# meco-group/omg-tools

Measured on AMD Instinct MI355X. Metric: MPC solves/sec, 1024-agent Holonomic Point2point batch per GPU, higher is better.
Workload: dtype f64

## Files before the change

### omg-tools_amd/csrc/omgx_core.h

```cpp
#pragma once
#include <stdint.h>
#include <math.h>

#ifdef OMGX_HOST_PORT
#define OMGX_FN inline
#define OMGX_HD inline
#else
#define OMGX_FN __device__ __forceinline__
#define OMGX_HD __host__ __device__ inline
#endif

#ifdef OMGX_HOST_PORT
#include <vector>
static thread_local std::vector<double> omgx_rbak;
#endif
#ifdef OMGX_COUNT_FACT
#include <atomic>
static std::atomic<long> omgx_dbg_nfact(0);
static std::atomic<long> omgx_dbg_cnt[12];
#endif
namespace omgx {

enum { ROW_FREE = 0, ROW_UPPER = 1, ROW_LOWER = 2, ROW_EQ = 3, ROW_BAD = 4 };
enum { OP_DIV = 0, OP_BSPL = 1, OP_COS = 2, OP_SIN = 3 };
// ... 207 lines not shown
  *lds = nl; *hbm = ng;
}

OMGX_HD size_t work_doubles(const Dims& d, int kkt_doubles) {
  size_t nl, ng;
  work_split(d, kkt_doubles, WS_LDS, &nl, &ng);
  return nl;
}

template <int MODE>
OMGX_HD void work_carve_split(Work& w, double* lds, double* hbm, const Dims& d, int kkt_doubles) {
  double* p = lds;
  double* g = hbm;
  w.slots = p; p += d.n_slots;
  if (!d.atoms_alias) { w.atoms = p; p += d.n_atoms; w.knots = p; p += d.n_knots; }
  w.x = p; p += d.N;             w.xt = p; p += d.N;
  w.gbar = p; p += d.N;          w.sol = p; p += d.N + d.n_eq;
  if (d.atoms_alias) { w.atoms = w.gbar; w.knots = w.gbar + d.n_atoms; }
  w.dinv = p; p += d.N;
  w.red = p; p += 64;
  if (ws_rows_hbm(MODE)) {
    w.ht = g; g += d.n_con;        w.rho = g; g += d.n_con;     w.vv = g; g += d.n_con;
    w.z = g; g += d.n_con;         w.ds = g; g += d.n_con;
    w.rtype = (int8_t*)g; g += (d.n_con + 7) / 8;
  } else {
    w.ht = p; p += d.n_con;        w.rho = p; p += d.n_con;     w.vv = p; p += d.n_con;
    w.z = p; p += d.n_con;         w.ds = p; p += d.n_con;
    w.rtype = (int8_t*)p; p += (d.n_con + 7) / 8;
  }
  if (ws_hv_hbm(MODE)) { w.hv = g; g += d.n_con; } else { w.hv = p; p += d.n_con; }
  if (ws_jac_hbm(MODE)) { w.jval = g; g += d.nnz_j + 1; } else { w.jval = p; p += d.nnz_j + 1; }
  if (ws_kkt_hbm(MODE)) { w.kkt = g; g += kkt_doubles; w.col = p; p += ws_root_lds(MODE) ? d.col_small : d.col_small_noroot; }
  else { w.kkt = p; p += kkt_doubles; w.col = p; p += d.col_doubles; }
  w.root = ws_root_lds(MODE) ? w.col + (OMGX_BMAT_DOUBLES + OMGX_STAGE_LD) * (OMGX_MAX_LEAF + 1) + OMGX_PAN_LD * (d.nr + 1) : nullptr;
}

OMGX_HD void work_carve(Work& w, double* base, const Dims& d, int kkt_doubles) {
  work_carve_split<WS_LDS>(w, base, nullptr, d, kkt_doubles);
}

#ifdef OMGX_HOST_PORT
struct Ctx {
  static constexpr bool wave_only = false, hbm = false, no_wave = false, root_lds = false, general = true, prep = false, refine = true, lean = false;
  double* red;
  int tid() const { return 0; }
  int nthr() const { return 1; }
  void sync() const {}
  double uni(double v) const { return v; }
  double rsum(double v) const { return v; }
  double wave_sum(double v) const { return v; }
  double rmax(double v) const { return v; }
  double rmin(double v) const { return v; }
  template <int... OPS> void reduce_ops(double (&)[sizeof...(OPS)]) const {}
  int lane() const { return 0; }
  int nlanes() const { return 1; }
  int wave() const { return 0; }
  int nwaves() const { return 1; }
  void wave_sync() const {}
};
#else
template <bool kHbm, bool kWaveOnly = false, bool kRootLds = false, bool kGeneral = false, bool kPrep = false, bool kRefine = false,
          bool kLean = false>
struct CtxT {
  static constexpr bool hbm = kHbm;
  static constexpr bool prep = kPrep;
  static constexpr bool refine = kRefine;
  static constexpr bool lean = kLean;
  static constexpr bool general = kGeneral;
  static constexpr bool root_lds = kRootLds;
  static constexpr bool wave_only = kWaveOnly;
  static constexpr bool no_wave = kHbm;
  double* red;
  long long* prof;
  __device__ int tid() const { int t = threadIdx.x; asm volatile("" : "+v"(t)); return t; }
  __device__ int nthr() const { return blockDim.x; }
  __device__ void sync() const { __syncthreads(); }
  template <int OP> static __device__ __forceinline__ double comb(double a, double b) {
    return OP == 0 ? a + b : (OP == 1 ? fmax(a, b) : fmin(a, b));
  }
  template <int OP, int CTRL> static __device__ __forceinline__ double dpp_comb(double v) {
    const int lo = __double2loint(v), hi = __double2hiint(v);
    const int lo2 = __builtin_amdgcn_update_dpp(lo, lo, CTRL, 0xf, 0xf, false);
    const int hi2 = __builtin_amdgcn_update_dpp(hi, hi, CTRL, 0xf, 0xf, false);
    return comb<OP>(v, __hiloint2double(hi2, lo2));
  }
  template <int OP> static __device__ __forceinline__ double wave_reduce(double v) {
    v = dpp_comb<OP, 0x128>(v);
    v = dpp_comb<OP, 0x124>(v);
    v = dpp_comb<OP, 0x122>(v);
    v = dpp_comb<OP, 0x121>(v);
    const double r0 = rl(v, 0), r1 = rl(v, 16), r2 = rl(v, 32), r3 = rl(v, 48);
    return comb<OP>(comb<OP>(r0, r1), comb<OP>(r2, r3));
  }
  static __device__ __forceinline__ double rl(double v, int lane) {
    return __hiloint2double(__builtin_amdgcn_readlane(__double2hiint(v), lane), __builtin_amdgcn_readlane(__double2loint(v), lane));
  }
  static __device__ __forceinline__ double uni(double v) {
    return __hiloint2double(__builtin_amdgcn_readfirstlane(__double2hiint(v)), __builtin_amdgcn_readfirstlane(__double2loint(v)));
  }
  template <int OP> __device__ double reduce(double v) const {
    v = wave_reduce<OP>(v);
    const int wave = threadIdx.x >> 6, nw = (blockDim.x + 63) >> 6;
    if ((threadIdx.x & 63) == 0) red[wave] = v;
    __syncthreads();
    double r = red[0];
    for (int i = 1; i < nw; ++i) r = comb<OP>(r, red[i]);
    __syncthreads();
    return uni(r);
  }
  template <int I, int N, int OP0, int... OPS>
  __device__ __forceinline__ void red_wave(double (&v)[N]) const {
    v[I] = wave_reduce<OP0>(v[I]);
    if ((threadIdx.x & 63) == 0) red[(threadIdx.x >> 6) * N + I] = v[I];
    if constexpr (sizeof...(OPS) > 0) red_wave<I + 1, N, OPS...>(v);
  }
  template <int I, int N, int OP0, int... OPS>
  __device__ __forceinline__ void red_block(double (&v)[N]) const {
    const int nw = (blockDim.x + 63) >> 6;
    double r = red[I];
    for (int k = 1; k < nw; ++k) r = comb<OP0>(r, red[k * N + I]);
    v[I] = uni(r);
    if constexpr (sizeof...(OPS) > 0) red_block<I + 1, N, OPS...>(v);
  }
  template <int... OPS> __device__ __forceinline__ void reduce_ops(double (&v)[sizeof...(OPS)]) const {
    static_assert(sizeof...(OPS) <= 8, "reduction scratch holds 8 values per wave");
    red_wave<0, sizeof...(OPS), OPS...>(v);
    __syncthreads();
    red_block<0, sizeof...(OPS), OPS...>(v);
    __syncthreads();
  }
  __device__ double rsum(double v) const { return reduce<0>(v); }
  __device__ double wave_sum(double v) const { return wave_reduce<0>(v); }
  __device__ double rmax(double v) const { return reduce<1>(v); }
  __device__ double rmin(double v) const { return reduce<2>(v); }
  __device__ int lane() const { return threadIdx.x & 63; }
  __device__ int nlanes() const { return 64; }
  __device__ int wave() const { return __builtin_amdgcn_readfirstlane(threadIdx.x >> 6); }
  __device__ int nwaves() const { return blockDim.x >> 6; }
  __device__ void wave_sync() const {
    if (kHbm) { __builtin_amdgcn_fence(__ATOMIC_RELEASE, "workgroup"); __builtin_amdgcn_wave_barrier(); __builtin_amdgcn_fence(__ATOMIC_ACQUIRE, "workgroup"); }
    else { __builtin_amdgcn_fence(__ATOMIC_RELEASE, "wavefront"); __builtin_amdgcn_wave_barrier(); __builtin_amdgcn_fence(__ATOMIC_ACQUIRE, "wavefront"); }
  }
};
typedef CtxT<false> Ctx;
#endif

#define OMGX_PFOR(i, n) for (int i = c.tid(); i < (n); i += c.nthr())
#define OMGX_PFOR_U4(i, n) _Pragma("unroll 4") for (int i = c.tid(); i < (n); i += c.nthr())

enum { PH_JAC = 0, PH_RESID, PH_ASSEMBLE, PH_FACTOR, PH_SOLVE, PH_STEP, PH_LINESEARCH, PH_UPDATE, PH_F_LEAF, PH_F_SCHUR, PH_F_ROOT, PH_LA, PH_LS, PH_LB, PH_SETUP, PH_TOTAL,
       PH_S_DESC, PH_S_PARAMS, PH_S_JAC0, PH_S_CLASS, PH_S_INIT, PH_A_ZERO, PH_A_PAIRS, PH_A_REST, PH_A_DIAG,
       PH_K_FWD, PH_K_ROOTRHS, PH_K_ROOT, PH_K_LEAFRHS, PH_K_BWD, PH_L_TERMS, PH_L_ROWS,
       PH_F_PARK, PH_F_SWEEP, PH_F_SCALE, PH_A_TCOL, PH_A_HESS, PH_P_LOAD, PH_P_DIV, PH_P_BSPL, PH_P_SLOTS, PH_COUNT };
#if defined(OMGX_PROFILE) && !defined(OMGX_HOST_PORT)
#define OMGX_TIC() long long tic_ = (c.sync(), clock64())
#define OMGX_TOC(k) do { c.sync(); long long now_ = clock64(); if (c.tid() == 0 && c.prof) c.prof[k] += now_ - tic_; tic_ = now_; } while (0)
#else
#define OMGX_TIC() do {} while (0)
#define OMGX_TOC(k) do {} while (0)
#endif

OMGX_FN double pp_eval(const Tables& T, int pp, const double* a) {
  double tot = 0.0;
  for (int m = T.pp_ptr[pp]; m < T.pp_ptr[pp + 1]; ++m) {
    double v = T.pm_coef[m];
    for (int q = T.pm_ptr[m]; q < T.pm_ptr[m + 1]; ++q) v *= a[T.pm_atom[q]];
    tot += v;
  }
  return tot;
}

OMGX_FN double csr_range_eval(const Tables& T, int m0, int m1, const double* a) {
  double tot = 0.0;
  for (int m = m0; m < m1; ++m) {
    double v = T.pm_coef[m];
    for (int q = T.pm_ptr[m]; q < T.pm_ptr[m + 1]; ++q) v *= a[T.pm_atom[q]];
    tot += v;
  }
  return tot;
}

OMGX_FN double mono_range_eval(const Tables& T, int m0, int m1, const double* a) {
  double tot = 0.0;
#pragma unroll 4
  for (int m = m0; m < m1; ++m) {
    const MonoRec r = T.pm_rec[m];
    double v = r.coef;
    if (r.a0 >= 0) { v *= a[r.a0]; if (r.a1 >= 0) { v *= a[r.a1]; if (r.a2 >= 0) { v *= a[r.a2]; if (r.a3 >= 0) v *= a[r.a3]; } } }
    tot += v;
  }
  return tot;
}

OMGX_FN double pp_eval_packed(const Tables& T, int pp, const double* a) {
  double tot = 0.0;
  const int m0 = T.pp_ptr[pp], m1 = T.pp_ptr[pp + 1];
#pragma unroll 4
  for (int m = m0; m < m1; ++m) {
    const MonoRec r = T.pm_rec[m];
    double v = r.coef;
    if (r.a0 >= 0) { v *= a[r.a0]; if (r.a1 >= 0) { v *= a[r.a1]; if (r.a2 >= 0) { v *= a[r.a2]; if (r.a3 >= 0) v *= a[r.a3]; } } }
    tot += v;
  }
  return tot;
}

template <bool GEN>
OMGX_FN void bspl_row(const double* k, int n_knots, int deg, double u, double* out) {
  const int n_fun = n_knots - deg - 1;
  int j = deg;
  for (int q = deg + 1; q < n_fun; ++q) if (k[q] < u) j = q;
  const bool inside = (u >= k[0]) && (u <= k[n_knots - 1]);
  if (GEN && deg > 5) {
    for (int i = 0; i < n_fun; ++i) out[i] = 0.0;
    if (!inside) return;
    double* Nv = out + (j - deg);
    Nv[0] = 1.0;
    for (int r = 1; r <= deg; ++r) {
      double saved = 0.0;
      for (int q = 0; q < r; ++q) {
        const double rgt = k[j + q + 1] - u, lft = u - k[j + 1 - (r - q)];
        const double den = rgt + lft;
        const double temp = den != 0.0 ? Nv[q] / den : 0.0;
        Nv[q] = saved + rgt * temp;
        saved = lft * temp;
      }
      Nv[r] = saved;
    }
    return;
  }
  double N[6], left[6], right[6];
#pragma unroll
  for (int r = 0; r < 6; ++r) { N[r] = 0.0; left[r] = 0.0; right[r] = 0.0; }
  N[0] = 1.0;
#pragma unroll
  for (int r = 1; r <= 5; ++r) {
    if (r <= deg) {
      left[r] = u - k[j + 1 - r];
      right[r] = k[j + r] - u;
      double saved = 0.0;
#pragma unroll
      for (int q = 0; q < 5; ++q) {
        if (q < r) {
          const double den = right[q + 1] + left[r - q];
          const double temp = den != 0.0 ? N[q] / den : 0.0;
          N[q] = saved + right[q + 1] * temp;
          saved = left[r - q] * temp;
        }
      }
      N[r] = saved;
    }
  }
  for (int i = 0; i < n_fun; ++i) out[i] = 0.0;
#pragma unroll
  for (int r = 0; r < 6; ++r) if (r <= deg && inside) out[j - deg + r] = N[r];
}

OMGX_FN double mono_value(const MonoRec& r, const double* at) {
  const double a0 = at[r.a0 < 0 ? 0 : r.a0], a1 = at[r.a1 < 0 ? 0 : r.a1];
  const double a2 = at[r.a2 < 0 ? 0 : r.a2], a3 = at[r.a3 < 0 ? 0 : r.a3];
  return r.coef * (r.a0 < 0 ? 1.0 : a0) * (r.a1 < 0 ? 1.0 : a1) * (r.a2 < 0 ? 1.0 : a2) * (r.a3 < 0 ? 1.0 : a3);
}
OMGX_FN double mono_value(const MonoRec8& r, const double* at) {
  const double a0 = at[r.a0 < 0 ? 0 : r.a0], a1 = at[r.a1 < 0 ? 0 : r.a1];
  const double a2 = at[r.a2 < 0 ? 0 : r.a2], a3 = at[r.a3 < 0 ? 0 : r.a3];
  const double a4 = at[r.a4 < 0 ? 0 : r.a4], a5 = at[r.a5 < 0 ? 0 : r.a5];
  const double a6 = at[r.a6 < 0 ? 0 : r.a6], a7 = at[r.a7 < 0 ? 0 : r.a7];
  return r.coef * (r.a0 < 0 ? 1.0 : a0) * (r.a1 < 0 ? 1.0 : a1) * (r.a2 < 0 ? 1.0 : a2) * (r.a3 < 0 ? 1.0 : a3)
                * (r.a4 < 0 ? 1.0 : a4) * (r.a5 < 0 ? 1.0 : a5) * (r.a6 < 0 ? 1.0 : a6) * (r.a7 < 0 ? 1.0 : a7);
}

template <class Rec, class C>
OMGX_FN void slots_packed(const C& c, const Dims& d, const Tables& T, Work& w) {
  const Rec* ell = (const Rec*)T.sl_ell;
  const Rec* rec = (const Rec*)T.pm_rec;
  OMGX_PFOR(i, d.n_slots) {
    const int L = T.sl_glen[i >> 6];
    double tot = 0.0;
    for (int s0 = 0; s0 < L; s0 += 4) {
      Rec q[4];
#pragma unroll
      for (int k = 0; k < 4; ++k) q[k] = ell[(s0 + k) * d.n_slots + i];
      double v[4];
#pragma unroll
      for (int k = 0; k < 4; ++k) v[k] = mono_value(q[k], w.atoms);
#pragma unroll
      for (int k = 0; k < 4; ++k) tot += v[k];
    }
    w.slots[T.sl_list[i]] = tot;
  }
  if (d.n_long > 0) {
    c.sync();
    for (int q = c.wave(); q < d.n_long; q += c.nwaves()) {
      const int sl = T.sl_list[q];
      const int m0 = T.slot_rng[2 * sl] + OMGX_SLOT_CAP, m1 = T.slot_rng[2 * sl + 1];
      double part = 0.0;
      for (int m = m0 + c.lane(); m < m1; m += c.nlanes()) part += mono_value(rec[m], w.atoms);
      const double rest = c.wave_sum(part);
      if (c.lane() == 0) w.slots[sl] += rest;
    }
  }
}

template <class C>
OMGX_FN void eval_params(const C& c, const Dims& d, const Tables& T, Work& w, const double* p) {
  OMGX_PFOR(i, d.n_par) w.atoms[i] = p[i];
  OMGX_TIC();
  OMGX_PFOR(i, d.n_knots) w.knots[i] = T.knots[i];
  c.sync();
  OMGX_TOC(PH_P_LOAD);
  for (int k = 0; k < d.n_prog;) {
    const int32_t* op = T.prog + 6 * k;
    if (op[0] != OP_BSPL) {
      if (c.tid() == 0) {
        const double num = d.mono_packed == 1 ? pp_eval_packed(T, op[1], w.atoms) : pp_eval(T, op[1], w.atoms);
        if (op[0] == OP_DIV) w.atoms[op[3]] = num / (d.mono_packed == 1 ? pp_eval_packed(T, op[2], w.atoms) : pp_eval(T, op[2], w.atoms));
        else if constexpr (C::general) w.atoms[op[3]] = op[0] == OP_COS ? cos(num) : sin(num);
      }
      ++k;
      c.sync();
      OMGX_TOC(PH_P_DIV);
      continue;
    } else {
      int k2 = k;
      while (k2 < d.n_prog && T.prog[6 * k2] == OP_BSPL) ++k2;
      OMGX_PFOR(it, k2 - k) {
        const int32_t* oq = T.prog + 6 * (k + it);
        bspl_row<C::general>(w.knots + oq[1], oq[2], oq[3], w.atoms[oq[4]], w.atoms + oq[5]);
      }
      k = k2;
    }
    c.sync();
    OMGX_TOC(PH_P_BSPL);
  }
  if (d.mono_packed == 1) slots_packed<MonoRec>(c, d, T, w);
  else if (d.mono_packed == 2) slots_packed<MonoRec8>(c, d, T, w);
  else {
    OMGX_PFOR(s, d.n_slots) {
      const int m0 = T.slot_rng[2 * s], m1 = T.slot_rng[2 * s + 1];
      w.slots[s] = csr_range_eval(T, m0, m1 < m0 + OMGX_SLOT_CAP ? m1 : m0 + OMGX_SLOT_CAP, w.atoms);
    }
    if (d.n_long > 0) {
      c.sync();
      for (int q = c.wave(); q < d.n_long; q += c.nwaves()) {
        const int sl = T.sl_list[q];
        const int m0 = T.slot_rng[2 * sl] + OMGX_SLOT_CAP, m1 = T.slot_rng[2 * sl + 1];
        double part = 0.0;
        for (int m = m0 + c.lane(); m < m1; m += c.nlanes()) part += csr_range_eval(T, m, m + 1, w.atoms);
        const double rest = c.wave_sum(part);
        if (c.lane() == 0) w.slots[sl] += rest;
      }
    }
  }
  c.sync();
  OMGX_TOC(PH_P_SLOTS);
}

OMGX_FN double term_coef(const Tables& T, const Work& w, int t) {
  const int sl = T.t_slot[t];
  return sl < 0 ? T.t_coef[t] : T.t_coef[t] * w.slots[sl];
}

OMGX_FN double rec_coef(const Work& w, double coef, int slot) { return slot < 0 ? coef : coef * w.slots[slot]; }

OMGX_FN double row_slack(const Work& w, int r, double t) { return t * w.vv[r] - w.hv[r]; }

template <bool Q4>
OMGX_FN double jitem_value(const JItem& q, const Work& w, const double* xv) {
  const double xs = w.slots[q.slot < 0 ? 0 : q.slot], xa = xv[q.va < 0 ? 0 : q.va], xb = xv[q.vb < 0 ? 0 : q.vb];
  double v = q.coef * (q.slot < 0 ? 1.0 : xs) * (q.va < 0 ? 1.0 : xa) * (q.vb < 0 ? 1.0 : xb);
  if (Q4) { const double xc = xv[q.vc < 0 ? 0 : q.vc]; v *= (q.vc < 0 ? 1.0 : xc); }
  return v;
}
#define OMGX_JE_OWN 4
template <class C, class F>
OMGX_FN void jac_entries4(const C& c, const JItem* ell, const int32_t* own, const int32_t* glen, int n_own, const Work& w, const double* xv, F fn) {
  OMGX_PFOR(o, n_own) {
    const int L = glen[o >> 6];
    int32_t er[OMGX_JE_OWN][2];
#pragma unroll
    for (int k = 0; k < OMGX_JE_OWN; ++k) { const int32_t* q = own + 2 * (k * n_own + o); er[k][0] = q[0]; er[k][1] = q[1]; }
    double sj[OMGX_JE_OWN];
    if (L == 1) {
      JItem q[OMGX_JE_OWN];
#pragma unroll
      for (int k = 0; k < OMGX_JE_OWN; ++k) q[k] = ell[k * n_own + o];
#pragma unroll
      for (int k = 0; k < OMGX_JE_OWN; ++k) sj[k] = jitem_value<C::general>(q[k], w, xv);
    } else {
#pragma unroll
      for (int k = 0; k < OMGX_JE_OWN; ++k) sj[k] = 0.0;
      for (int s0 = 0; s0 < L; s0 += 2) {
        JItem q[2 * OMGX_JE_OWN];
#pragma unroll
        for (int k = 0; k < 2 * OMGX_JE_OWN; ++k) q[k] = ell[(s0 * OMGX_JE_OWN + k) * n_own + o];
        double v[2 * OMGX_JE_OWN];
#pragma unroll
        for (int k = 0; k < 2 * OMGX_JE_OWN; ++k) v[k] = jitem_value<C::general>(q[k], w, xv);
#pragma unroll
        for (int k = 0; k < OMGX_JE_OWN; ++k) { sj[k] += v[k]; sj[k] += v[OMGX_JE_OWN + k]; }
      }
    }
#pragma unroll
    for (int k = 0; k < OMGX_JE_OWN; ++k) if (er[k][0] >= 0) fn(er[k][0], er[k][1], sj[k]);
  }
}

#define OMGX_ROW_BATCH 8
template <bool Q4>
OMGX_FN double row_value_ell_t(const Tables& T, const Work& w, int i, int m, const double* xv) {
  const int L = T.rt_glen[i >> 6];
  double g = 0.0;
  for (int s0 = 0; s0 < L; s0 += OMGX_ROW_BATCH) {
    RowTerm q[OMGX_ROW_BATCH];
#pragma unroll
    for (int k = 0; k < OMGX_ROW_BATCH; ++k) q[k] = T.rt_ell[(s0 + k) * m + i];
    double v[OMGX_ROW_BATCH];
#pragma unroll
    for (int k = 0; k < OMGX_ROW_BATCH; ++k) {
      const double xs = w.slots[q[k].slot < 0 ? 0 : q[k].slot];
      const double x0 = xv[q[k].v0 < 0 ? 0 : q[k].v0], x1 = xv[q[k].v1 < 0 ? 0 : q[k].v1], x2 = xv[q[k].v2 < 0 ? 0 : q[k].v2];
      v[k] = q[k].coef * (q[k].slot < 0 ? 1.0 : xs) * (q[k].v0 < 0 ? 1.0 : x0) * (q[k].v1 < 0 ? 1.0 : x1) * (q[k].v2 < 0 ? 1.0 : x2);
      if (Q4) { const double x3 = xv[q[k].v3 < 0 ? 0 : q[k].v3]; v[k] *= (q[k].v3 < 0 ? 1.0 : x3); }
    }
#pragma unroll
    for (int k = 0; k < OMGX_ROW_BATCH; ++k) g += v[k];
  }
  return g;
}
template <class C>
OMGX_FN double row_value_ell(const Dims& d, const Tables& T, const Work& w, int i, int m, const double* xv) {
  return row_value_ell_t<C::general>(T, w, i, m, xv);
}

template <class C>
OMGX_FN void lift_project(const C& c, const Dims& d, const Tables& T, const Work& w, int m, double* xv) {
  if (d.n_lift == 0) return;
  for (int L = 0; L < d.lift_depth; ++L) {
    const int k0 = T.lift_lev[L], k1 = T.lift_lev[L + 1];
    OMGX_PFOR(kk, k1 - k0) {
      const int32_t* q = T.lift_rec + 2 * (k0 + kk);
      xv[q[1]] = 0.0;
      const double g0 = row_value_ell<C>(d, T, w, q[0], m, xv);
      xv[q[1]] = 1.0;
      const double g1 = row_value_ell<C>(d, T, w, q[0], m, xv);
      const double den = g1 - g0;
      xv[q[1]] = den != 0.0 ? -g0 / den : NAN;
    }
    c.sync();
  }
}

template <class C>
OMGX_FN double row_value_share(const C& c, const Tables& T, const Work& w, int r, const double* xv) {
  double g = 0.0;
  for (int t = T.row_ptr[r] + c.tid(); t < T.row_ptr[r + 1]; t += c.nthr()) {
    double v = term_coef(T, w, t);
    const int32_t* tv = T.t_var + OMGX_TV * t;
    for (int k = 0; k < OMGX_TV && tv[k] >= 0; ++k) v *= xv[tv[k]];
    g += v;
  }
  return g;
}

OMGX_FN int tri(int i, int k) { return i * (i + 1) / 2 + k; }

struct Kkt {
  const int32_t *d_off, *b_off, *leaf_off, *leaf_bw, *cpl_ptr, *cpl_idx, *blk, *cpl_map, *lf_w, *lf_ldb, *lf_band, *lf_kind, *dl_pos;
  int n_leaf, n_root, root_off;
  double* a;
  OMGX_FN void bind(const Dims& dd, const Tables& TT, double* store) {
    d_off = TT.d_off; b_off = TT.b_off; leaf_off = TT.leaf_off; leaf_bw = TT.leaf_bw; cpl_ptr = TT.cpl_ptr;
    cpl_idx = TT.cpl_idx; blk = TT.blk; cpl_map = TT.cpl_map;
    lf_w = TT.lf_w; lf_ldb = TT.lf_ldb; lf_band = TT.lf_band; lf_kind = TT.lf_kind; dl_pos = TT.dl_pos;
    n_leaf = dd.n_leaf; n_root = dd.n_root; root_off = dd.root_off; a = store;
  }
  OMGX_FN double* P(int l) const { return a + d_off[l]; }
  OMGX_FN int ld(int l) const { return b_off[l]; }
  OMGX_FN double* R() const { return a + d_off[n_leaf]; }
  OMGX_FN int nl(int l) const { return leaf_off[l + 1] - leaf_off[l]; }
  OMGX_FN int nc(int l) const { return cpl_ptr[l + 1] - cpl_ptr[l]; }
};

struct BMat { int a, ld, nfact, rows, npos, dinv, pan, cpl, bw, pad_; };
static_assert(sizeof(BMat) <= OMGX_BMAT_DOUBLES * sizeof(double), "BMat larger than its LDS slot");
#define OMGX_NB 4
#define OMGX_PAN_SMALL(n) (4 * (n) + 16)

#define OMGX_PANEL_STRIDES(C, M, sr, sc) const int sr = C::hbm ? 1 : (M).ld, sc = C::hbm ? (M).ld : 1
OMGX_FN int baddr(const BMat& M, int r, int k) { return M.a + r * M.ld + (M.ld == 0 ? 1 : 0) * ((r * (r + 1)) >> 1) + k; }
template <int KIND>
OMGX_FN int baddr_k(const BMat& M, int r, int k) {
  return KIND == 1 ? M.a + r * M.ld + k : (KIND == 2 ? M.a + ((r * (r + 1)) >> 1) + k : baddr(M, r, k));
}

#ifdef OMGX_HOST_PORT
OMGX_FN double rcp_pivot(double d) { return 1.0 / d; }
#else
OMGX_FN double rcp_pivot(double d) {
  double y = __builtin_amdgcn_rcp(d);
  y = fma(fma(-d, y, 1.0), y, y);
  y = fma(fma(-d, y, 1.0), y, y);
  return y;
}
#endif

}
#ifndef OMGX_HOST_PORT
#include "omgx_wave.h"
#endif
namespace omgx {

struct Blk4 { double l10, l20, l21, l30, l31, l32, d0, d1, d2, d3, i0, i1, i2, i3; };
OMGX_FN Blk4 blk4_from(double g00, double g10, double g11, double g20, double g21, double g22,
                       double g30, double g31, double g32, double g33) {
  Blk4 b;
  b.d0 = g00; b.i0 = rcp_pivot(b.d0);
  b.l10 = g10 * b.i0; b.l20 = g20 * b.i0; b.l30 = g30 * b.i0;
  b.d1 = g11 - b.l10 * g10; b.i1 = rcp_pivot(b.d1);
  const double w21 = g21 - g20 * b.l10, w31 = g31 - g30 * b.l10;
  b.l21 = w21 * b.i1; b.l31 = w31 * b.i1;
  b.d2 = g22 - b.l20 * g20 - b.l21 * w21; b.i2 = rcp_pivot(b.d2);
  const double w32 = g32 - g30 * b.l20 - w31 * b.l21;
  b.l32 = w32 * b.i2;
  b.d3 = g33 - b.l30 * g30 - b.l31 * w31 - b.l32 * w32; b.i3 = rcp_pivot(b.d3);
  return b;
}

template <int KIND>
OMGX_FN Blk4 blk4_factor(const BMat& M, const double* A, int jb, int nb) {
  double g[4][4];
#pragma unroll
  for (int a = 0; a < 4; ++a)
#pragma unroll
    for (int k = 0; k <= a; ++k) {
      const double v = A[baddr_k<KIND>(M, jb + (a < nb ? a : 0), jb + (a < nb ? k : 0))];
      g[a][k] = (a < nb) ? v : (a == k ? 1.0 : 0.0);
    }
  return blk4_from(g[0][0], g[1][0], g[1][1], g[2][0], g[2][1], g[2][2], g[3][0], g[3][1], g[3][2], g[3][3]);
}

template <class C>
OMGX_FN void ldl_left4(const C& c, const BMat* Ms, int nm, double* A, double* dinvb, double* colb, int* bad) {
  int nmax = 0, total_rows = 0, total_blocks = 0;
  for (int i = 0; i < nm; ++i) {
    if (Ms[i].nfact > nmax) nmax = Ms[i].nfact;
    total_rows += Ms[i].rows; total_blocks += (Ms[i].nfact + 3) >> 2;
  }
  OMGX_TIC();
  OMGX_PFOR(it, total_blocks * 10) {
    int mi = 0, blk = it / 10; const int e = it - 10 * blk;
    while (blk >= ((Ms[mi].nfact + 3) >> 2)) { blk -= (Ms[mi].nfact + 3) >> 2; ++mi; }
    const BMat M = Ms[mi];
    const int a = e < 1 ? 0 : (e < 3 ? 1 : (e < 6 ? 2 : 3)), k = e - ((a * (a + 1)) >> 1);
    const int ra = 4 * blk + a, ck = 4 * blk + k;
    OMGX_PANEL_STRIDES(C, M, sr, sc);
    colb[M.pan + M.nfact + 10 * blk + e] = (ra < M.nfact) ? A[M.a + ra * sr + ck * sc] : (a == k ? 1.0 : 0.0);
  }
  c.sync();
  OMGX_TOC(PH_F_PARK);
  int badl = 0;
  for (int jb = 0; jb < nmax; jb += OMGX_NB) {
    OMGX_PFOR(it, total_rows) {
      int mi = 0, r = it;
      while (r >= Ms[mi].rows) { r -= Ms[mi].rows; ++mi; }
      const BMat M = Ms[mi];
      if (jb >= M.nfact || r < jb) continue;
      const int nb = (M.nfact - jb) < OMGX_NB ? (M.nfact - jb) : OMGX_NB;
      double* iv = (M.dinv >= 0) ? dinvb + M.dinv : colb + M.pan;
      const double* db = colb + M.pan + M.nfact + 10 * (jb >> 2);
      const bool diag_row = r < jb + nb;
      const int q1 = nb > 1 ? 1 : 0, q2 = nb > 2 ? 2 : 0, q3 = nb > 3 ? 3 : 0;
      OMGX_PANEL_STRIDES(C, M, sr, sc);
      const int b0 = M.a + jb * sr, b1 = M.a + (jb + q1) * sr, b2 = M.a + (jb + q2) * sr, b3 = M.a + (jb + q3) * sr;
      const int br = M.a + r * sr;
      double g00 = db[0], g10 = db[1], g11 = db[2], g20 = db[3], g21 = db[4], g22 = db[5],
             g30 = db[6], g31 = db[7], g32 = db[8], g33 = db[9];
      double v0 = A[br + jb * sc], v1 = A[br + (jb + q1) * sc], v2 = A[br + (jb + q2) * sc], v3 = A[br + (jb + q3) * sc];
      const double m1 = nb > 1 ? 1.0 : 0.0, m2 = nb > 2 ? 1.0 : 0.0, m3 = nb > 3 ? 1.0 : 0.0;
      const int k0 = jb > M.bw ? jb - M.bw : 0;
#pragma unroll 4
      for (int k = k0; k < jb; ++k) {
        const double tk = iv[k];
        const double u0 = A[b0 + k * sc], u1 = m1 * A[b1 + k * sc], u2 = m2 * A[b2 + k * sc], u3 = m3 * A[b3 + k * sc], ur = A[br + k * sc];
        const double t0 = u0 * tk, t1 = u1 * tk, t2 = u2 * tk, t3 = u3 * tk;
        g00 -= u0 * t0;
        g10 -= u1 * t0; g11 -= u1 * t1;
        g20 -= u2 * t0; g21 -= u2 * t1; g22 -= u2 * t2;
        g30 -= u3 * t0; g31 -= u3 * t1; g32 -= u3 * t2; g33 -= u3 * t3;
        v0 -= ur * t0; v1 -= ur * t1; v2 -= ur * t2; v3 -= ur * t3;
      }
      const Blk4 B = blk4_from(g00, g10, g11, g20, g21, g22, g30, g31, g32, g33);
      if (diag_row) {
        const int q = r - jb;
        const double dq = q == 0 ? B.d0 : (q == 1 ? B.d1 : (q == 2 ? B.d2 : B.d3));
        const double iq = q == 0 ? B.i0 : (q == 1 ? B.i1 : (q == 2 ? B.i2 : B.i3));
        const bool pos_ok = (jb + q < M.npos) ? (dq > 0.0) : (dq < 0.0);
        if (!pos_ok) badl = 1;
        iv[jb + q] = iq;
        if (q == 1) { A[br + jb * sc] = B.l10 * B.d0; }
        else if (q == 2) { A[br + jb * sc] = B.l20 * B.d0; A[br + (jb + 1) * sc] = B.l21 * B.d1; }
        else if (q == 3) { A[br + jb * sc] = B.l30 * B.d0; A[br + (jb + 1) * sc] = B.l31 * B.d1; A[br + (jb + 2) * sc] = B.l32 * B.d2; }
        A[br + (jb + q) * sc] = dq;
      } else {
        const double u0 = v0;
        const double u1 = v1 - u0 * B.l10;
        const double u2 = v2 - u0 * B.l20 - u1 * B.l21;
        const double u3 = v3 - u0 * B.l30 - u1 * B.l31 - u2 * B.l32;
        A[br + jb * sc] = u0;
        if (nb > 1) A[br + (jb + 1) * sc] = u1;
        if (nb > 2) A[br + (jb + 2) * sc] = u2;
        if (nb > 3) A[br + (jb + 3) * sc] = u3;
      }
    }
    c.sync();
  }
  OMGX_TOC(PH_F_SWEEP);
  *bad = c.rmax(badl ? 1.0 : 0.0) > 0.0 ? 1 : 0;
  OMGX_TOC(PH_F_SCALE);
}

#ifndef OMGX_HOST_PORT
template <int KIND, class C>
OMGX_FN void ldl_left4_coop(const C& c, const BMat* Ms, int nm, double* A, double* dinvb, double* colb, int* bad,
                            int total_rows, int nmax) {
  const int lane = c.lane(), wave = c.wave();
  const int row_waves = (total_rows + 63) >> 6;
  const bool is_row = c.tid() < total_rows;
  const bool is_blk = wave >= row_waves && wave < row_waves + nm;
  int r = c.tid();
  BMat M = Ms[0];
  if (is_row) { int mi = 0; while (r >= Ms[mi].rows) { r -= Ms[mi].rows; ++mi; } M = Ms[mi]; }
  else if (is_blk) { M = Ms[wave - row_waves]; r = -1; }
  double* iv = (M.dinv >= 0) ? dinvb + M.dinv : colb + M.pan;
  double* gb = colb + M.pan + M.nfact;
  double* bb = gb + 16;
// ... 1868 lines not shown
```

Measured before the change: 3.288 million.

## Fuse scalar DIV op with following B-spline run to drop a barrier

The parameter program interpreter now groups each non-BSPL op (DIV/COS/SIN) with the run of BSPL ops that follows it and executes both in one phase. Threads whose B-spline row depends on the scalar result recompute it redundantly instead of waiting for thread 0 and a block barrier. Non-dependent rows read the atom directly. This removes one block-wide sync per scalar op, at the cost of duplicated scalar evaluation across dependent threads and a more intricate dependency check that assumes BSPL rows only depend on the immediately preceding op.

```diff
diff --git a/omg-tools_amd/csrc/omgx_core.h b/omg-tools_amd/csrc/omgx_core.h
--- a/omg-tools_amd/csrc/omgx_core.h
+++ b/omg-tools_amd/csrc/omgx_core.h
@@ -533,36 +533,42 @@
   }
 }
 
+struct ProgRun { int kd, k2; };
+OMGX_FN ProgRun prog_scan(const Dims& d, const Tables& T, int k) {
+  ProgRun r;
+  r.kd = (k < d.n_prog && T.prog[6 * k] != OP_BSPL) ? k + 1 : k;
+  r.k2 = r.kd;
+  if (r.kd == k || T.prog[6 * k] == OP_DIV) { while (r.k2 < d.n_prog && T.prog[6 * r.k2] == OP_BSPL) ++r.k2; }
+  return r;
+}
+
 template <class C>
 OMGX_FN void eval_params(const C& c, const Dims& d, const Tables& T, Work& w, const double* p) {
   OMGX_PFOR(i, d.n_par) w.atoms[i] = p[i];
   OMGX_TIC();
   OMGX_PFOR(i, d.n_knots) w.knots[i] = T.knots[i];
+  ProgRun run = prog_scan(d, T, 0);
   c.sync();
   OMGX_TOC(PH_P_LOAD);
-  for (int k = 0; k < d.n_prog;) {
-    const int32_t* op = T.prog + 6 * k;
-    if (op[0] != OP_BSPL) {
-      if (c.tid() == 0) {
+  for (int k = 0; k < d.n_prog; run = prog_scan(d, T, k)) {
+    const int nb = run.k2 - run.kd, nd = run.kd - k;
+    for (int it = c.nthr() - 1 - c.tid(); it < nb + nd; it += c.nthr()) {
+      const bool row = it < nb;
+      const int32_t* oq = T.prog + 6 * (row ? run.kd + it : k);
+      const bool own = !row || (nd > 0 && T.prog[6 * k + 3] == oq[4]);
+      double u = 0.0;
+      if (own) {
+        const int32_t* op = T.prog + 6 * k;
         const double num = d.mono_packed == 1 ? pp_eval_packed(T, op[1], w.atoms) : pp_eval(T, op[1], w.atoms);
-        if (op[0] == OP_DIV) w.atoms[op[3]] = num / (d.mono_packed == 1 ? pp_eval_packed(T, op[2], w.atoms) : pp_eval(T, op[2], w.atoms));
-        else if constexpr (C::general) w.atoms[op[3]] = op[0] == OP_COS ? cos(num) : sin(num);
-      }
-      ++k;
-      c.sync();
-      OMGX_TOC(PH_P_DIV);
-      continue;
-    } else {
-      int k2 = k;
-      while (k2 < d.n_prog && T.prog[6 * k2] == OP_BSPL) ++k2;
-      OMGX_PFOR(it, k2 - k) {
-        const int32_t* oq = T.prog + 6 * (k + it);
-        bspl_row<C::general>(w.knots + oq[1], oq[2], oq[3], w.atoms[oq[4]], w.atoms + oq[5]);
-      }
-      k = k2;
-    }
+        if (op[0] == OP_DIV) u = num / (d.mono_packed == 1 ? pp_eval_packed(T, op[2], w.atoms) : pp_eval(T, op[2], w.atoms));
+        else if constexpr (C::general) u = op[0] == OP_COS ? cos(num) : sin(num);
+      } else u = w.atoms[oq[4]];
+      if (row) bspl_row<C::general>(w.knots + oq[1], oq[2], oq[3], u, w.atoms + oq[5]);
+      else w.atoms[oq[3]] = u;
+    }
+    k = run.k2;
     c.sync();
-    OMGX_TOC(PH_P_BSPL);
+    OMGX_TOC(nd > 0 ? PH_P_DIV : PH_P_BSPL);
   }
   if (d.mono_packed == 1) slots_packed<MonoRec>(c, d, T, w);
   else if (d.mono_packed == 2) slots_packed<MonoRec8>(c, d, T, w);
```

New measurement: 3.288 million, median of 2. No clear change (-0.0%).
